# deweylab/RSEM

Measured on AMD Instinct MI355X. Metric: EM read-alignments/s (nnz x EM iterations per second), rsem-run-em theta-only rounds, higher is better.
Workload: dtype f64; 1 GPU; BASELINE configs[2] (PairedEndQModel-shaped, the north-star target config): EM matrix of 50000000 reads x 200000 transcripts, 570042118 alignments (11.40/read) per GPU, frozen conprb (rounds >= 12); synthetic_config=C3, kernel=0, parallelism=1 GPU

## Files before the change

### rsem_amd/csrc/estep_block.hpp

```cpp
#pragma once
#include <type_traits>

#include "simt_macros.hpp"

RSEM_DEVFN double wave_sum(double v) {
#pragma unroll
    for (int d = 32; d >= 1; d >>= 1) v += RSEM_SHFL_XOR(v, d);
    return v;
}


struct ThetaSrc {
    const double* v;
    double extra0, sum;
};
template <bool kFC>
RSEM_DEVFN double theta_at(const ThetaSrc& t, int i) {
    if (!kFC) return t.v[i];
    return (t.v[i] + (i == 0 ? t.extra0 : 0.0)) / t.sum;
}
template <bool kFC>
RSEM_DEVFN ThetaSrc theta_src(const double* __restrict__ v, const double* __restrict__ tsrc, double N0, int lane);

template <bool kFC>
RSEM_DEVFN void stage_windows(int base, int span, int M, const ThetaSrc& th, double* th_win, double* cnt_win) {
    for (int i = RSEM_TIDX; i < span; i += RSEM_BDIM) {
        const int sidv = base + i;
        th_win[i] = (sidv >= 0 && sidv <= M) ? theta_at<kFC>(th, sidv) : 0.0;
        cnt_win[i] = 0.0;
    }
    RSEM_SYNC();
}

struct XArgs {
    const double* extra = nullptr;
    double* inv = nullptr;
    uint32_t slot_base = 0;
};

#ifndef RSEM_FARQ_CAP
#define RSEM_FARQ_CAP 384
#endif
constexpr int kFarQCap = RSEM_FARQ_CAP;
static_assert(kFarQCap > 256, "a slice of K = 4 planes can append 256 entries");
struct FarQueue {
    int* sid = nullptr;
    double* val = nullptr;
    int* n = nullptr;
};

struct StartList {
    const int32_t* list = nullptr;
    const uint32_t* off = nullptr;
};

template <int K, bool kQ>
struct SliceRegs {
    int id[K];
    typename std::conditional<kQ, uint32_t, double>::type c[K];
    double nc;
    int e;
    double x;
    uint32_t slot0;
    double traw[K];
};

RSEM_DEVFN double pow2_of(int e) { return RSEM_LL_AS_DOUBLE((long long)(1023 + e) << 52); }

#ifndef RSEM_F64_DEPTHS
#define RSEM_F64_DEPTHS 2, 2, 2, 2
#endif
#ifndef RSEM_Q32_DEPTHS
#define RSEM_Q32_DEPTHS 2, 2, 2, 2
#endif
template <typename T>
RSEM_DEVFN T stream_load(const T* p) { return RSEM_NT_LOAD(p); }
template <int kCtrl>
RSEM_DEVFN double dpp_take(double v) {
    const long long b = RSEM_DOUBLE_AS_LL(v);
    const int lo = RSEM_DPP_MOV((int)(unsigned)b, kCtrl);
    const int hi = RSEM_DPP_MOV((int)(unsigned)(b >> 32), kCtrl);
    return RSEM_LL_AS_DOUBLE(((long long)hi << 32) | (unsigned)lo);
}
RSEM_DEVFN double read_sum_dpp(double part, int lg) {
    if (lg >= 1) part += dpp_take<0xB1>(part);
    if (lg >= 2) part += dpp_take<0x4E>(part);
    if (lg >= 3) part += dpp_take<0x141>(part);
    if (lg >= 4) part += dpp_take<0x140>(part);
    for (int d = 16; d < (1 << lg); d <<= 1) part += RSEM_SHFL_XOR(part, d);
    return part;
}
constexpr int kF64Depth[4] = {RSEM_F64_DEPTHS};
constexpr int kQ32Depth[4] = {RSEM_Q32_DEPTHS};

template <int K, bool kFC, bool kQ, int NBUF, bool kFar, bool kX = false, bool kFQ = false>
RSEM_DEVFN void estep_block(const Shape& S, uint32_t s_begin, uint32_t s_end, int lane, int base, int span,
                                   const double* __restrict__ theta, const double* __restrict__ tsrc, double N0, double* th_win, double* cnt_win,
                                   const unsigned char* __restrict__ sval, const int16_t* __restrict__ sexp, const int32_t* __restrict__ ssid,
                                   const double* __restrict__ sncp, const unsigned long long* __restrict__ masks,
                                   double* counts, double& noise, double& neff, int M, const XArgs& X = XArgs(), const FarQueue& FQ = FarQueue(),
                                   const StartList& SL = StartList()) {
    static_assert(!kFQ || kFar, "the far queue belongs to the loop of the units with ids outside their window");
    static_assert(!kFQ || NBUF >= 3, "the far-queue loop requests theta a slice ahead: three register sets at least (the ring loop)");
    using ValT = typename std::conditional<kQ, uint32_t, double>::type;
    const ValT* __restrict__ scp = (const ValT*)(sval + S.val_base);
    const int lg = S.lg;
    const int g = lane & ((1 << lg) - 1);
    const bool g0 = (g == 0);
    const uint32_t R = 64u >> lg;
    const bool kList = !kFQ && SL.list != nullptr;
    uint32_t m_base = s_begin;
    unsigned long long mv = (s_begin + lane < s_end) ? masks[s_begin + lane] : ~0ull;
    uint32_t ov = 0;
    if (kList) ov = (s_begin + lane < s_end) ? SL.off[s_begin + lane] : 0u;
    auto mask_of = [&](uint32_t t) -> unsigned long long {
        if (t - m_base >= 64u) {
            m_base = t;
            mv = (t + lane < s_end) ? masks[t + lane] : ~0ull;
            if (kList) { ov = (t + lane < s_end) ? SL.off[t + lane] : 0u; RSEM_PIN(ov); }
            RSEM_PIN(mv);
        }
        const int src = (int)(t - m_base);
        const uint32_t lo = RSEM_READLANE((int)(uint32_t)mv, src);
        const uint32_t hi = RSEM_READLANE((int)(uint32_t)(mv >> 32), src);
        return ((unsigned long long)hi << 32) | lo;
    };
    const unsigned ulane = (unsigned)lane, uslot = ulane >> lg;
    const unsigned Gk = (unsigned)shape_Gk(S);
    const unsigned last_lane = uslot * Gk + ((unsigned)g < Gk ? (unsigned)g : Gk - 1u);
    const bool last_ok = (unsigned)g < Gk;
    const uint32_t vstride = (uint32_t)RSEM_READFIRSTLANE((int)shape_val_stride(S));
    auto issue = [&](uint32_t t, unsigned long long m, SliceRegs<K, kQ>& b) {
        const uint32_t sl = t - S.slice_base;
        const uint64_t v0 = (uint64_t)sl * (K * 64);
        const ValT* __restrict__ vp = scp + (uint64_t)sl * vstride;
        if (kFQ || m != 0ull) {
            const int32_t* __restrict__ ip = ssid + (S.plane_base * 64 + v0);
            unsigned stride = 64u, idx = ulane;
            if (!kFQ) {
                const bool from_list = kList && t != s_begin;
                if (from_list) {
                    const uint32_t off = (uint32_t)RSEM_READLANE((int)ov, (int)(t - m_base));
                    const unsigned n = (unsigned)__builtin_popcountll(m);
                    const unsigned rank = (unsigned)RSEM_MBCNT((uint32_t)m, (uint32_t)(m >> 32));
                    ip = SL.list + off;
                    stride = n;
                    idx = rank < n ? rank : n - 1u;
                }
            }
#pragma unroll
            for (int k = 0; k < K; k++) b.id[k] = ip[(unsigned)k * stride + idx];
        }
#pragma unroll
        for (int k = 0; k < K - 1; k++) b.c[k] = stream_load(&vp[k * 64 + ulane]);
        b.c[K - 1] = stream_load(&vp[(K - 1) * 64 + last_lane]);
        const uint32_t slot0 = S.slot_base + sl * R;
        b.nc = (sncp + slot0)[uslot];
        b.e = kQ ? (int)(sexp + slot0)[uslot] : 0;
        b.x = kX ? (X.extra + (slot0 - X.slot_base))[uslot] : 0.0;
        b.slot0 = slot0;
    };
    auto spill = [&](const int* rsid, double* acc) {
#pragma unroll
        for (int k = 0; k < K; k++) {
            if (acc[k] != 0.0) {
                const unsigned off = (unsigned)(rsid[k] - base);
                if (!kFar) RSEM_LDS_ADD(&cnt_win[off < (unsigned)span ? off : 0u], acc[k]);
                else if (off < (unsigned)span) RSEM_LDS_ADD(&cnt_win[off], acc[k]);
                else if (kFQ) {
                    const int at = RSEM_LDS_FETCH_ADD_I32(FQ.n, 1);
                    FQ.sid[at] = rsid[k];
                    FQ.val[at] = acc[k];
                } else RSEM_ATOMIC_ADD(&counts[rsid[k]], acc[k]);
            }
            acc[k] = 0.0;
        }
    };
    auto far_queue_room = [&](bool all) {
        if (!kFQ) return;
        RSEM_WAVE_SYNC();
        const int n = RSEM_READFIRSTLANE(*FQ.n);
        if (n > (all ? 0 : kFarQCap - 64 * K)) {
            for (int i = lane; i < n; i += 64) RSEM_ATOMIC_ADD(&counts[FQ.sid[i]], FQ.val[i]);
            RSEM_WAIT_VM0();
            RSEM_WAVE_SYNC();
            if (lane == 0) *FQ.n = 0;
            RSEM_WAVE_SYNC();
        }
    };

    int rsid[K];
    double rth[K], acc[K];
#pragma unroll
    for (int k = 0; k < K; k++) { rsid[k] = 0; rth[k] = 0.0; acc[k] = 0.0; }
    ThetaSrc th{theta, 0.0, 1.0};
    double th0 = 0.0;
    auto pregather = [&](SliceRegs<K, kQ>& b, unsigned long long m) {
        if (!kFQ) return;
        const bool starts = ((m >> lane) & 1ull) != 0ull;
#pragma unroll
        for (int k = 0; k < K; k++) {
            const int sidv = b.id[k];
            const bool want = starts && !((unsigned)(sidv - base) < (unsigned)span);
            b.traw[k] = th.v[want ? sidv : 0];
        }
    };
    auto reduce = [&](const SliceRegs<K, kQ>& cur, unsigned long long cur_m) {
        if (cur_m != 0ull) {
            far_queue_room(false);
            if ((cur_m >> lane) & 1ull) {
                spill(rsid, acc);
                bool far = false;
#pragma unroll
                for (int k = 0; k < K; k++) {
                    const int sidv = cur.id[k];
                    rsid[k] = sidv;
                    const unsigned off = (unsigned)(sidv - base);
                    const bool in = off < (unsigned)span;
                    rth[k] = th_win[in ? off : 0u];
                    far = far || !in;
                }
                if (kFQ) {
#pragma unroll
                    for (int k = 0; k < K; k++)
                        if (!((unsigned)(rsid[k] - base) < (unsigned)span))
                            rth[k] = kFC ? (cur.traw[k] + (rsid[k] == 0 ? th.extra0 : 0.0)) / th.sum : cur.traw[k];
                } else if (kFar && far) {
                    double t[K];
#pragma unroll
                    for (int k = 0; k < K; k++) {
                        const bool in = (unsigned)(rsid[k] - base) < (unsigned)span;
                        t[k] = theta_at<kFC>(th, in ? 0 : rsid[k]);
                    }
#pragma unroll
                    for (int k = 0; k < K; k++) {
                        RSEM_PIN(t[k]);
                        if (!((unsigned)(rsid[k] - base) < (unsigned)span)) rth[k] = t[k];
                    }
                }
            }
        }
        double f0 = g0 ? th0 * cur.nc : 0.0;
        if (f0 < kEpsilon) f0 = 0.0;
        double f[K];
        double part = f0 + ((kX && g0) ? cur.x : 0.0);
        const double scale = kQ ? pow2_of(cur.e) : 1.0;
#pragma unroll
        for (int k = 0; k < K; k++) {
            const ValT cr = (k == K - 1 && !last_ok) ? ValT(0) : cur.c[k];
            const double cv = kQ ? (double)cr * scale : (double)cr;
            double v = rth[k] * cv;
            if (v < kEpsilon) v = 0.0;
            f[k] = v;
            part += v;
        }
        part = read_sum_dpp(part, lg);
        const double inv = (part >= kEpsilon) ? 1.0 / part : 0.0;
        if (kX) RSEM_STORE_SAME(&(X.inv + (cur.slot0 - X.slot_base))[uslot], inv);
        noise += f0 * inv;
        neff += (g0 && part >= kEpsilon) ? 1.0 : 0.0;
#pragma unroll
        for (int k = 0; k < K; k++) acc[k] = acc[k] + f[k] * inv;
    };
    if constexpr (NBUF == 2) {
        SliceRegs<K, kQ> A, B;
        unsigned long long mA = ~0ull, mB = 0;
        issue(s_begin, mA, A);
        th = theta_src<kFC>(theta, tsrc, N0, lane);
        th0 = theta_at<kFC>(th, 0);
        stage_windows<kFC>(base, span, M, th, th_win, cnt_win);
        uint32_t s = s_begin;
        for (; s + 2 < s_end; s += 2) {
            mB = mask_of(s + 1);
            issue(s + 1, mB, B);
            reduce(A, mA);
            mA = mask_of(s + 2);
            issue(s + 2, mA, A);
            reduce(B, mB);
        }
        if (s + 1 < s_end) {
            mB = mask_of(s + 1);
            issue(s + 1, mB, B);
            reduce(A, mA);
            reduce(B, mB);
        } else {
            reduce(A, mA);
        }
    } else {
        SliceRegs<K, kQ> buf[NBUF];
        unsigned long long mk[NBUF];
        mk[0] = ~0ull;
        issue(s_begin, mk[0], buf[0]);
        th = theta_src<kFC>(theta, tsrc, N0, lane);
        th0 = theta_at<kFC>(th, 0);
        stage_windows<kFC>(base, span, M, th, th_win, cnt_win);
        auto within = [&](uint32_t t) -> uint32_t { return t < s_end ? t : s_end - 1u; };
#pragma unroll
        for (int j = 1; j < NBUF - 1; j++) {
            const uint32_t tt = within(s_begin + j);
            mk[j] = mask_of(tt);
            issue(tt, mk[j], buf[j]);
        }
        pregather(buf[0], mk[0]);
        uint32_t s = s_begin;
        for (; s + NBUF <= s_end; s += NBUF) {
#pragma unroll
            for (int j = 0; j < NBUF; j++) {
                constexpr int ahead = NBUF - 1;
                const int nj = (j + ahead) % NBUF;
                const uint32_t tt = within(s + j + ahead);
                mk[nj] = mask_of(tt);
                issue(tt, mk[nj], buf[nj]);
                pregather(buf[(j + 1) % NBUF], mk[(j + 1) % NBUF]);
                reduce(buf[j], mk[j]);
            }
        }
#pragma unroll
        for (int j = 0; j < NBUF - 1; j++)
            if (s + j < s_end) {
                if (j > 0) pregather(buf[j], mk[j]);
                reduce(buf[j], mk[j]);
            }
    }
    far_queue_room(false);
    spill(rsid, acc);
    far_queue_room(true);
}

template <bool kFC>
RSEM_DEVFN ThetaSrc theta_src(const double* __restrict__ v, const double* __restrict__ tsrc, double N0, int lane) {
    ThetaSrc t{v, 0.0, 1.0};
    if (kFC) {
        const double a = wave_sum(tsrc[lane]);
        const double b = wave_sum(tsrc[kTotSlots + lane]);
        t.extra0 = a + N0;
        t.sum = b + N0;
    }
    return t;
}
```

### rsem_amd/csrc/simt_macros.hpp

```cpp
#pragma once
#ifndef RSEM_EMU
#define RSEM_DEVFN __device__ inline
#define RSEM_TIDX ((int)threadIdx.x)
#define RSEM_BDIM ((int)blockDim.x)
#define RSEM_SYNC() __syncthreads()
#define RSEM_SHFL_XOR(v, d) __shfl_xor(v, d)
#define RSEM_SHFL_DOWN(v, d) __shfl_down(v, d)
#define RSEM_SHFL_UP(v, d) __shfl_up(v, d)
#define RSEM_SHFL(v, src) __shfl(v, src)
#define RSEM_BALLOT(p) __ballot(p)
#define RSEM_READLANE(v, src) __builtin_amdgcn_readlane(v, src)
#define RSEM_ATOMIC_ADD(p, v) unsafeAtomicAdd(p, v)
#define RSEM_ATOMIC_ADD_I32(p, v) atomicAdd(p, v)
#define RSEM_LDS_ADD(p, v) (void)__builtin_amdgcn_ds_atomic_fadd_f64((__attribute__((address_space(3))) double*)(p), v)
#define RSEM_LDS_ADD_I32(p, v) (void)__hip_atomic_fetch_add((__attribute__((address_space(3))) int*)(p), v, __ATOMIC_RELAXED, __HIP_MEMORY_SCOPE_WORKGROUP)
#define RSEM_LDS_FETCH_ADD_I32(p, v) __hip_atomic_fetch_add((__attribute__((address_space(3))) int*)(p), v, __ATOMIC_RELAXED, __HIP_MEMORY_SCOPE_WORKGROUP)
#define RSEM_WAVE_SYNC()                                        \
    do {                                                        \
        __builtin_amdgcn_fence(__ATOMIC_RELEASE, "wavefront");  \
        __builtin_amdgcn_wave_barrier();                        \
        __builtin_amdgcn_fence(__ATOMIC_ACQUIRE, "wavefront");  \
    } while (0)
#define RSEM_WAIT_VM0() __builtin_amdgcn_s_waitcnt(0x0F70)
#define RSEM_READFIRSTLANE(v) __builtin_amdgcn_readfirstlane(v)
#define RSEM_MBCNT(lo, hi) __builtin_amdgcn_mbcnt_hi(hi, __builtin_amdgcn_mbcnt_lo(lo, 0u))
#define RSEM_PIN(x) asm volatile("" : "+v"(x))
#define RSEM_SCHED_FENCE() __builtin_amdgcn_sched_barrier(0)
#define RSEM_RCP(x) __builtin_amdgcn_rcp(x)
#define RSEM_DPP_MOV(v, ctrl) __builtin_amdgcn_update_dpp(0, v, ctrl, 0xf, 0xf, false)
#define RSEM_LL_AS_DOUBLE(x) __longlong_as_double(x)
#define RSEM_DOUBLE_AS_LL(x) __double_as_longlong(x)
#define RSEM_STORE_SAME(p, v) (*(p) = (v))
#define RSEM_NT_LOAD(p) __builtin_nontemporal_load(p)
#define RSEM_AGENT_LOAD(p) __hip_atomic_load(p, __ATOMIC_RELAXED, __HIP_MEMORY_SCOPE_AGENT)
#define RSEM_AGENT_STORE(p, v) __hip_atomic_store(p, v, __ATOMIC_RELAXED, __HIP_MEMORY_SCOPE_AGENT)
#define RSEM_AGENT_EXCHANGE(p, v) __hip_atomic_exchange(p, v, __ATOMIC_RELAXED, __HIP_MEMORY_SCOPE_AGENT)
#define RSEM_AGENT_FETCH_ADD(p, v) __hip_atomic_fetch_add(p, v, __ATOMIC_RELAXED, __HIP_MEMORY_SCOPE_AGENT)
#define RSEM_AGENT_FETCH_MAX(p, v) __hip_atomic_fetch_max(p, v, __ATOMIC_RELAXED, __HIP_MEMORY_SCOPE_AGENT)
#define RSEM_HOST_RELEASE_STORE(p, v) __hip_atomic_store(p, v, __ATOMIC_RELEASE, __HIP_MEMORY_SCOPE_SYSTEM)
#define RSEM_ZERO_DEP(z, x) asm volatile("v_and_b32 %0, 0, %1" : "=v"(z) : "v"(x))
#else
#ifndef RSEM_MBCNT
#define RSEM_MBCNT(lo, hi) __builtin_popcountll((((unsigned long long)(hi) << 32) | (unsigned long long)(lo)) & ((1ull << emu::lane()) - 1ull))
#endif
#endif
```

Before: 666.2 billion read-alignments/s.

## Trim per-slice E-step overhead: running pointers, ballot-gated clamp, wave-level neff count

Several micro-optimizations land together in the E-step block. Per-slice address recomputation is replaced with running pointers that advance each issue. The read-sum DPP chain is nested under a scalar-pinned lg, and DPP moves set bound_ctrl. The epsilon clamp now runs only when a wave-wide ballot finds any small nonzero term, and the last-lane zeroing moves to the theta gather. The neff accumulation becomes a scalar popcount of ballots added once at the end. Together these cut VALU instruction count in the hot reduce loop, but they alter subtle semantics (f0 clamping, last_ok masking, masking last_lane to 63) that could cause correctness divergence.

```diff
diff --git a/rsem_amd/csrc/estep_block.hpp b/rsem_amd/csrc/estep_block.hpp
--- a/rsem_amd/csrc/estep_block.hpp
+++ b/rsem_amd/csrc/estep_block.hpp
@@ -83,11 +83,20 @@
     return RSEM_LL_AS_DOUBLE(((long long)hi << 32) | (unsigned)lo);
 }
 RSEM_DEVFN double read_sum_dpp(double part, int lg) {
-    if (lg >= 1) part += dpp_take<0xB1>(part);
-    if (lg >= 2) part += dpp_take<0x4E>(part);
-    if (lg >= 3) part += dpp_take<0x141>(part);
-    if (lg >= 4) part += dpp_take<0x140>(part);
-    for (int d = 16; d < (1 << lg); d <<= 1) part += RSEM_SHFL_XOR(part, d);
+    RSEM_PIN_S(lg);
+    if (lg >= 1) {
+        part += dpp_take<0xB1>(part);
+        if (lg >= 2) {
+            part += dpp_take<0x4E>(part);
+            if (lg >= 3) {
+                part += dpp_take<0x141>(part);
+                if (lg >= 4) {
+                    part += dpp_take<0x140>(part);
+                    for (int d = 16; d < (1 << lg); d <<= 1) part += RSEM_SHFL_XOR(part, d);
+                }
+            }
+        }
+    }
     return part;
 }
 constexpr int kF64Depth[4] = {RSEM_F64_DEPTHS};
@@ -127,18 +136,23 @@
     };
     const unsigned ulane = (unsigned)lane, uslot = ulane >> lg;
     const unsigned Gk = (unsigned)shape_Gk(S);
-    const unsigned last_lane = uslot * Gk + ((unsigned)g < Gk ? (unsigned)g : Gk - 1u);
+    const unsigned last_lane = (uslot * Gk + ((unsigned)g < Gk ? (unsigned)g : Gk - 1u)) & 63u;
     const bool last_ok = (unsigned)g < Gk;
     const uint32_t vstride = (uint32_t)RSEM_READFIRSTLANE((int)shape_val_stride(S));
-    auto issue = [&](uint32_t t, unsigned long long m, SliceRegs<K, kQ>& b) {
-        const uint32_t sl = t - S.slice_base;
-        const uint64_t v0 = (uint64_t)sl * (K * 64);
-        const ValT* __restrict__ vp = scp + (uint64_t)sl * vstride;
+    const uint32_t sl_begin = s_begin - S.slice_base;
+    const ValT* __restrict__ vrun = scp + (uint64_t)sl_begin * vstride;
+    const int32_t* __restrict__ irun = kFQ ? ssid + (S.plane_base * 64 + (uint64_t)sl_begin * (K * 64)) : nullptr;
+    uint32_t slot_run = S.slot_base + sl_begin * R;
+    const double* __restrict__ nrun = sncp + slot_run;
+    const int16_t* __restrict__ erun = kQ ? sexp + slot_run : nullptr;
+    const double* __restrict__ xrun = kX ? X.extra + (slot_run - X.slot_base) : nullptr;
+    auto issue = [&](uint32_t t, unsigned long long m, SliceRegs<K, kQ>& b, bool first, bool advance) {
+        const ValT* __restrict__ vp = vrun;
         if (kFQ || m != 0ull) {
-            const int32_t* __restrict__ ip = ssid + (S.plane_base * 64 + v0);
+            const int32_t* __restrict__ ip = kFQ ? irun : ssid + (S.plane_base * 64 + (uint64_t)(t - S.slice_base) * (K * 64));
             unsigned stride = 64u, idx = ulane;
             if (!kFQ) {
-                const bool from_list = kList && t != s_begin;
+                const bool from_list = kList && !(first && t == s_begin);
                 if (from_list) {
                     const uint32_t off = (uint32_t)RSEM_READLANE((int)ov, (int)(t - m_base));
                     const unsigned n = (unsigned)__builtin_popcountll(m);
@@ -153,12 +167,19 @@
         }
 #pragma unroll
         for (int k = 0; k < K - 1; k++) b.c[k] = stream_load(&vp[k * 64 + ulane]);
-        b.c[K - 1] = stream_load(&vp[(K - 1) * 64 + last_lane]);
-        const uint32_t slot0 = S.slot_base + sl * R;
-        b.nc = (sncp + slot0)[uslot];
-        b.e = kQ ? (int)(sexp + slot0)[uslot] : 0;
-        b.x = kX ? (X.extra + (slot0 - X.slot_base))[uslot] : 0.0;
-        b.slot0 = slot0;
+        b.c[K - 1] = stream_load(&(vp + (K - 1) * 64)[last_lane]);
+        b.nc = nrun[uslot];
+        b.e = kQ ? (int)erun[uslot] : 0;
+        b.x = kX ? xrun[uslot] : 0.0;
+        b.slot0 = slot_run;
+        if (advance) {
+            vrun += vstride;
+            if (kFQ) irun += K * 64;
+            slot_run += R;
+            nrun += R;
+            if (kQ) erun += R;
+            if (kX) xrun += R;
+        }
     };
     auto spill = [&](const int* rsid, double* acc) {
 #pragma unroll
@@ -195,6 +216,8 @@
     for (int k = 0; k < K; k++) { rsid[k] = 0; rth[k] = 0.0; acc[k] = 0.0; }
     ThetaSrc th{theta, 0.0, 1.0};
     double th0 = 0.0;
+    const unsigned long long g0_lanes = RSEM_BALLOT(g0);
+    int n_mass = 0;
     auto pregather = [&](SliceRegs<K, kQ>& b, unsigned long long m) {
         if (!kFQ) return;
         const bool starts = ((m >> lane) & 1ull) != 0ull;
@@ -238,49 +261,57 @@
                         if (!((unsigned)(rsid[k] - base) < (unsigned)span)) rth[k] = t[k];
                     }
                 }
-            }
-        }
-        double f0 = g0 ? th0 * cur.nc : 0.0;
-        if (f0 < kEpsilon) f0 = 0.0;
+                if (!last_ok) rth[K - 1] = 0.0;
+            }
+        }
+        double f0 = th0 * cur.nc;
         double f[K];
-        double part = f0 + ((kX && g0) ? cur.x : 0.0);
+        bool clamp = (f0 < kEpsilon) & (f0 != 0.0);
         const double scale = kQ ? pow2_of(cur.e) : 1.0;
 #pragma unroll
         for (int k = 0; k < K; k++) {
-            const ValT cr = (k == K - 1 && !last_ok) ? ValT(0) : cur.c[k];
-            const double cv = kQ ? (double)cr * scale : (double)cr;
-            double v = rth[k] * cv;
-            if (v < kEpsilon) v = 0.0;
-            f[k] = v;
-            part += v;
-        }
+            const double cv = kQ ? (double)cur.c[k] * scale : (double)cur.c[k];
+            f[k] = rth[k] * cv;
+            clamp |= (f[k] < kEpsilon) & (f[k] != 0.0);
+        }
+        if (RSEM_BALLOT(clamp) != 0ull) {
+            RSEM_PIN(f0);
+            if (f0 < kEpsilon) f0 = 0.0;
+#pragma unroll
+            for (int k = 0; k < K; k++)
+                if (f[k] < kEpsilon) f[k] = 0.0;
+        }
+        double part = kX ? f0 + (g0 ? cur.x : 0.0) : f0;
+#pragma unroll
+        for (int k = 0; k < K; k++) part += f[k];
         part = read_sum_dpp(part, lg);
-        const double inv = (part >= kEpsilon) ? 1.0 / part : 0.0;
+        const bool mass = part >= kEpsilon;
+        const double inv = mass ? 1.0 / part : 0.0;
         if (kX) RSEM_STORE_SAME(&(X.inv + (cur.slot0 - X.slot_base))[uslot], inv);
         noise += f0 * inv;
-        neff += (g0 && part >= kEpsilon) ? 1.0 : 0.0;
+        n_mass += __builtin_popcountll(RSEM_BALLOT(mass) & g0_lanes);
 #pragma unroll
         for (int k = 0; k < K; k++) acc[k] = acc[k] + f[k] * inv;
     };
     if constexpr (NBUF == 2) {
         SliceRegs<K, kQ> A, B;
         unsigned long long mA = ~0ull, mB = 0;
-        issue(s_begin, mA, A);
+        issue(s_begin, mA, A, true, true);
         th = theta_src<kFC>(theta, tsrc, N0, lane);
-        th0 = theta_at<kFC>(th, 0);
+        th0 = g0 ? theta_at<kFC>(th, 0) : 0.0;
         stage_windows<kFC>(base, span, M, th, th_win, cnt_win);
         uint32_t s = s_begin;
         for (; s + 2 < s_end; s += 2) {
             mB = mask_of(s + 1);
-            issue(s + 1, mB, B);
+            issue(s + 1, mB, B, false, true);
             reduce(A, mA);
             mA = mask_of(s + 2);
-            issue(s + 2, mA, A);
+            issue(s + 2, mA, A, false, true);
             reduce(B, mB);
         }
         if (s + 1 < s_end) {
             mB = mask_of(s + 1);
-            issue(s + 1, mB, B);
+            issue(s + 1, mB, B, false, true);
             reduce(A, mA);
             reduce(B, mB);
         } else {
@@ -290,16 +321,16 @@
         SliceRegs<K, kQ> buf[NBUF];
         unsigned long long mk[NBUF];
         mk[0] = ~0ull;
-        issue(s_begin, mk[0], buf[0]);
+        issue(s_begin, mk[0], buf[0], true, s_begin + 1u < s_end);
         th = theta_src<kFC>(theta, tsrc, N0, lane);
-        th0 = theta_at<kFC>(th, 0);
+        th0 = g0 ? theta_at<kFC>(th, 0) : 0.0;
         stage_windows<kFC>(base, span, M, th, th_win, cnt_win);
         auto within = [&](uint32_t t) -> uint32_t { return t < s_end ? t : s_end - 1u; };
 #pragma unroll
         for (int j = 1; j < NBUF - 1; j++) {
             const uint32_t tt = within(s_begin + j);
             mk[j] = mask_of(tt);
-            issue(tt, mk[j], buf[j]);
+            issue(tt, mk[j], buf[j], true, tt + 1u < s_end);
         }
         pregather(buf[0], mk[0]);
         uint32_t s = s_begin;
@@ -310,7 +341,7 @@
                 const int nj = (j + ahead) % NBUF;
                 const uint32_t tt = within(s + j + ahead);
                 mk[nj] = mask_of(tt);
-                issue(tt, mk[nj], buf[nj]);
+                issue(tt, mk[nj], buf[nj], true, tt + 1u < s_end);
                 pregather(buf[(j + 1) % NBUF], mk[(j + 1) % NBUF]);
                 reduce(buf[j], mk[j]);
             }
@@ -325,6 +356,7 @@
     far_queue_room(false);
     spill(rsid, acc);
     far_queue_room(true);
+    neff += (lane == 0) ? (double)n_mass : 0.0;
 }
 
 template <bool kFC>
diff --git a/rsem_amd/csrc/simt_macros.hpp b/rsem_amd/csrc/simt_macros.hpp
--- a/rsem_amd/csrc/simt_macros.hpp
+++ b/rsem_amd/csrc/simt_macros.hpp
@@ -25,9 +25,10 @@
 #define RSEM_READFIRSTLANE(v) __builtin_amdgcn_readfirstlane(v)
 #define RSEM_MBCNT(lo, hi) __builtin_amdgcn_mbcnt_hi(hi, __builtin_amdgcn_mbcnt_lo(lo, 0u))
 #define RSEM_PIN(x) asm volatile("" : "+v"(x))
+#define RSEM_PIN_S(x) asm volatile("; uniform value pinned" : "+s"(x))
 #define RSEM_SCHED_FENCE() __builtin_amdgcn_sched_barrier(0)
 #define RSEM_RCP(x) __builtin_amdgcn_rcp(x)
-#define RSEM_DPP_MOV(v, ctrl) __builtin_amdgcn_update_dpp(0, v, ctrl, 0xf, 0xf, false)
+#define RSEM_DPP_MOV(v, ctrl) __builtin_amdgcn_update_dpp(0, v, ctrl, 0xf, 0xf, true)
 #define RSEM_LL_AS_DOUBLE(x) __longlong_as_double(x)
 #define RSEM_DOUBLE_AS_LL(x) __double_as_longlong(x)
 #define RSEM_STORE_SAME(p, v) (*(p) = (v))
@@ -43,4 +44,7 @@
 #ifndef RSEM_MBCNT
 #define RSEM_MBCNT(lo, hi) __builtin_popcountll((((unsigned long long)(hi) << 32) | (unsigned long long)(lo)) & ((1ull << emu::lane()) - 1ull))
 #endif
+#ifndef RSEM_PIN_S
+#define RSEM_PIN_S(x) (void)(x)
 #endif
+#endif
```

Result: no change. 665.6 billion read-alignments/s (-0.1%).
